# guanjq/targetdiff

Measured on NVIDIA H100. Metric: molecules/sec (1000-step sampling, CrossDocked pocket shape), higher is better.
Workload: dtype f32 (storage, LayerNorm, softmax, accumulation); GEMM operands as 2-piece bf16 splits on wgmma (3 products, ~16-bit operand mantissa)

## Files before the change

targetdiff_b200/csrc/edge_mlp_v4.cu:

```cuda
#include <stdio.h>
#include <stdlib.h>
#include <string.h>

#include "tdiff_common.cuh"
#include "hopper_mma.cuh"

namespace v4 {

constexpr int kCons = 2;
constexpr int kThreads = (kCons + 1) * 128;
constexpr int kTile = 64;
constexpr int kTabClassBytes = 2 * 128 * 128;
constexpr int kProdRegs = 40, kConsRegs = 232;
constexpr int kSrcStride = 512 + 32, kDst = 8;
constexpr int sSrc = 0, sDstRows = sSrc + kTile * kSrcStride, sMeta = sDstRows + kDst * 512, kStage = sMeta + kTile * 16;
constexpr int kMAtom = 32 * 128, kMPiece = 2 * kMAtom, kMImg = 2 * kMPiece;
template <bool FOLD>
struct Map {
  static constexpr int W = 0, T = W + 4 * 128 * 128, Par = T + (FOLD ? 1 : 2) * kTabClassBytes, X = Par + 2 * 128 * 4,
                       M = X + kCons * 4 * 2 * 128 * 4, C = M + (FOLD ? kCons * kMImg : 0), Stage = C + (FOLD ? kCons * 32 * 4 : 0),
                       Bar = Stage + kCons * kStage, Smem = Bar + 8 * (1 + 2 * kCons);
  static_assert(M % 1024 == 0 && Stage % 128 == 0 && kStage % 128 == 0 && Smem <= 227 * 1024, "shared-memory map");
};
constexpr int kOrderBar = 5;
constexpr int kFoldBar = 7;

__device__ __forceinline__ uint32_t smem_u32(const void* p) { return (uint32_t)__cvta_generic_to_shared(p); }
__device__ __forceinline__ void mbar_init(uint32_t bar, uint32_t count) {
  asm volatile("mbarrier.init.shared::cta.b64 [%0], %1;" ::"r"(bar), "r"(count) : "memory");
}
__device__ __forceinline__ void mbar_wait(uint32_t bar, uint32_t parity) {
  asm volatile(
      "{\n\t.reg .pred p;\n\tWAIT_LOOP:\n\tmbarrier.try_wait.parity.shared::cta.b64 p, [%0], %1;\n\t@p bra WAIT_DONE;\n\tbra WAIT_LOOP;\n\t"
      "WAIT_DONE:\n\t}" ::"r"(bar), "r"(parity) : "memory");
}
__device__ __forceinline__ void mbar_expect_tx(uint32_t bar, uint32_t bytes) {
  asm volatile("mbarrier.arrive.expect_tx.shared::cta.b64 _, [%0], %1;" ::"r"(bar), "r"(bytes) : "memory");
}
__device__ __forceinline__ void bulk_g2s(uint32_t smem_dst, const void* gsrc, uint32_t bytes, uint32_t bar) {
  asm volatile("cp.async.bulk.shared::cluster.global.mbarrier::complete_tx::bytes [%0], [%1], %2, [%3];" ::"r"(smem_dst), "l"(gsrc), "r"(bytes),
               "r"(bar) : "memory");
}
__device__ __forceinline__ void fence_barrier_init() { asm volatile("fence.mbarrier_init.release.cluster;" ::: "memory"); }
__device__ __forceinline__ void mbar_arrive(uint32_t bar) { asm volatile("mbarrier.arrive.shared::cta.b64 _, [%0];" ::"r"(bar) : "memory"); }
__device__ __forceinline__ void mbar_expect_tx_only(uint32_t bar, uint32_t bytes) {
  asm volatile("mbarrier.expect_tx.shared::cta.b64 [%0], %1;" ::"r"(bar), "r"(bytes) : "memory");
}
__device__ __forceinline__ void named_bar_sync(int id, int nthreads) { asm volatile("bar.sync %0, %1;" ::"r"(id), "r"(nthreads) : "memory"); }
__device__ __forceinline__ void named_bar_arrive(int id, int nthreads) { asm volatile("bar.arrive %0, %1;" ::"r"(id), "r"(nthreads) : "memory"); }
template <int N> __device__ __forceinline__ void setmaxnreg_inc() { asm volatile("setmaxnreg.inc.sync.aligned.u32 %0;" ::"n"(N)); }
template <int N> __device__ __forceinline__ void setmaxnreg_dec() { asm volatile("setmaxnreg.dec.sync.aligned.u32 %0;" ::"n"(N)); }

__device__ __forceinline__ uint32_t cvt_bf16x2(float hi, float lo) {
  uint32_t d;
  asm("cvt.rn.bf16x2.f32 %0, %1, %2;" : "=r"(d) : "f"(hi), "f"(lo));
  return d;
}
__device__ __forceinline__ float ex2_approx(float x) { float y; asm("ex2.approx.ftz.f32 %0, %1;" : "=f"(y) : "f"(x)); return y; }
__device__ __forceinline__ void stg64(float* p, float a, float b) { asm volatile("st.global.v2.f32 [%0], {%1,%2};" ::"l"(p), "f"(a), "f"(b) : "memory"); }
__device__ __forceinline__ void stg128(float* p, float a, float b, float c, float d) {
  asm volatile("st.global.v4.f32 [%0], {%1,%2,%3,%4};" ::"l"(p), "f"(a), "f"(b), "f"(c), "f"(d) : "memory");
}

struct LnParams { float b[128]; float b2[128]; float mu[20]; };
struct AggArgs {
  const float* logits;
  const float* e_w;
  float* h;
  int key_softmax;
};

template <int N, int M, int LO_BIT>
__device__ __forceinline__ void transpose_reduce(float (&t)[N], int lane) {
  if constexpr (N > M) {
    constexpr int h = (N / M / 2) << LO_BIT;
    const bool up = lane & h;
#pragma unroll
    for (int i = 0; i < N / 2; ++i) {
      const float send = up ? t[i] : t[i + N / 2];
      const float keep = up ? t[i + N / 2] : t[i];
      t[i] = keep + __shfl_xor_sync(0xffffffffu, send, h);
    }
    transpose_reduce<N / 2, M, LO_BIT>(reinterpret_cast<float(&)[N / 2]>(t), lane);
  }
}
__device__ __forceinline__ void split2(float y0, float y1, uint32_t& hi, uint32_t& lo) {
  hi = cvt_bf16x2(y1, y0);
  const float r0 = __fsub_rn(y0, __uint_as_float(hi << 16)), r1 = __fsub_rn(y1, __uint_as_float(hi & 0xffff0000u));
  lo = cvt_bf16x2(r1, r0);
}

}

using namespace v4;

template <int NOUT, bool FOLD>
__global__ void __launch_bounds__(kThreads, 1)
edge_mlp_v4_kernel(const float* __restrict__ P, int zero_row, const int* __restrict__ src, const unsigned char* __restrict__ etype,
                   const float* __restrict__ dist_arr, const int* __restrict__ row_nodes, long long n_dst, long long split_dst,
                   const int* __restrict__ d_counts, int k, int offA, int offB, const unsigned char* __restrict__ w2_image,
                   const unsigned char* __restrict__ tab_image, float coeff, const float* __restrict__ qnode, float* __restrict__ out, int out_by_slot, AggArgs agg,
                   int fold_cls, const __grid_constant__ LnParams lp) {
  static_assert(!FOLD || NOUT == 128, "the fold applies to the key MLPs");
  using L = Map<FOLD>;
  extern __shared__ __align__(1024) unsigned char smem_raw[];
  const uint32_t sbase = smem_u32(smem_raw);
  const uint32_t sW = sbase + L::W, sT = sbase + L::T, sBar = sbase + L::Bar;
  float* const s_b = reinterpret_cast<float*>(smem_raw + L::Par);
  float* const s_b2 = s_b + 128;
  const int tid = threadIdx.x, lane = tid & 31, warp = __shfl_sync(0xffffffffu, tid >> 5, 0);
  const int w = warp & 3, q = lane & 3;
  const int kshift = (k & (k - 1)) == 0 ? __ffs(k) - 1 : -1;
  auto row_dst = [&](long long idx, int& j) -> unsigned {
    const unsigned a = kshift >= 0 ? (unsigned)idx >> kshift : (unsigned)idx / (unsigned)k;
    j = (int)((unsigned)idx - a * (unsigned)k);
    return a;
  };

  if ((sbase & 1023u) != 0) __trap();
  if (d_counts) { n_dst = d_counts[0]; split_dst = d_counts[1]; }
  const long long n_rows = n_dst * k, split_rows = split_dst * k;
  long long row_lo = 0, row_hi = n_rows;
  if constexpr (FOLD) { if (fold_cls) row_lo = split_rows; else row_hi = split_rows; }
  const long long n_tiles = row_hi > row_lo ? (row_hi - row_lo + kTile - 1) / kTile : 0;
  const long long my_tiles = (n_tiles > blockIdx.x) ? (n_tiles - blockIdx.x + gridDim.x - 1) / gridDim.x : 0;
  auto full_bar = [&](int c) { return sBar + 8u * (1 + c); };
  auto empty_bar = [&](int c) { return sBar + 8u * (1 + kCons + c); };

  constexpr int kWAtom = NOUT * 128;
  constexpr int kWPiece = 2 * kWAtom;
  if (tid == 0) {
    mbar_init(sBar, 1);
    for (int c = 0; c < kCons; ++c) { mbar_init(full_bar(c), 32); mbar_init(empty_bar(c), 128); }
    fence_barrier_init();
    if constexpr (FOLD) {
      mbar_expect_tx(sBar, 4u * 128 * 128 + kTabClassBytes);
      bulk_g2s(sW, w2_image, 4u * 128 * 128, sBar);
      bulk_g2s(sT, tab_image + (size_t)fold_cls * kTabClassBytes, kTabClassBytes, sBar);
    } else {
      mbar_expect_tx(sBar, 2u * kWPiece + 2u * kTabClassBytes);
      bulk_g2s(sW, w2_image, 2u * kWPiece, sBar);
      bulk_g2s(sT, tab_image, 2u * kTabClassBytes, sBar);
    }
  }
  for (int i = tid; i < 128; i += kThreads) { s_b[i] = lp.b[i]; s_b2[i] = lp.b2[i]; }
  __syncthreads();

  if (warp < 4) {
    setmaxnreg_dec<kProdRegs>();
    if (warp >= kCons) return;
    const int c = warp;
    const uint32_t st = sbase + L::Stage + (uint32_t)c * kStage;
    for (long long it = c, use = 0; it < my_tiles; it += kCons, ++use) {
      const long long tile = blockIdx.x + it * (long long)gridDim.x, row0 = row_lo + tile * kTile;
      int j0;
      const unsigned a0 = row_dst(row0, j0);
      const long long last = (row0 + kTile - 1 < row_hi ? row0 + kTile - 1 : row_hi - 1);
      const int n_d = min(kDst, (int)(row_dst(last, j0) - a0) + 1);
      int s[2];
      int4 meta[2];
#pragma unroll
      for (int h = 0; h < 2; ++h) {
        const long long idx = row0 + lane + 32 * h;
        int jj = 0, ty = 3, slot = 0, node = -1;
        float dist = 0.f;
        s[h] = -1;
        if (idx < n_rows) {
          const unsigned a = row_dst(idx, jj);
          slot = a - a0 < (unsigned)kDst ? (int)(a - a0) + 1 : 0;
          node = row_nodes[a];
          if (node >= 0) {
            const size_t e = (size_t)node * k + jj;
            s[h] = src[e]; ty = etype[e]; dist = dist_arr[e];
          }
        }
        meta[h] = make_int4(node, s[h], __float_as_int(dist), ty | (slot << 8) | (jj << 16));
      }
      int dnode = -1;
      if (lane < n_d) dnode = row_nodes[a0 + lane];
      mbar_wait(empty_bar(c), (uint32_t)(use & 1) ^ 1u);
#pragma unroll
      for (int h = 0; h < 2; ++h) *reinterpret_cast<int4*>(smem_raw + L::Stage + c * kStage + sMeta + 16 * (lane + 32 * h)) = meta[h];
      if (lane == 0) mbar_expect_tx_only(full_bar(c), (uint32_t)(kTile + (FOLD ? 2 : 1) * n_d) * 512u);
      __syncwarp();
#pragma unroll
      for (int h = 0; h < 2; ++h)
        bulk_g2s(st + sSrc + (uint32_t)(lane + 32 * h) * kSrcStride, P + (size_t)(s[h] >= 0 ? s[h] : zero_row) * TD_NPROJ + offB, 512u, full_bar(c));
      if (lane < n_d) bulk_g2s(st + sDstRows + (uint32_t)lane * 512u, P + (size_t)(dnode >= 0 ? dnode : zero_row) * TD_NPROJ + offA, 512u, full_bar(c));
      if (FOLD && lane < n_d) bulk_g2s(st + sDstRows + (uint32_t)(2 + lane) * 512u, qnode + (size_t)(dnode >= 0 ? dnode : 0) * TD_H, 512u, full_bar(c));
      mbar_arrive(full_bar(c));
    }
    return;
  }

  setmaxnreg_inc<kConsRegs>();
  const int cwg = (warp >> 2) - 1;
  float mu[5];
#pragma unroll
  for (int m = 0; m < 5; ++m) mu[m] = lp.mu[5 * q + m];
  const float coeff2 = coeff * 1.4426950408889634f;
  mbar_wait(sBar, 0);

  const int r_base = 16 * w + (lane >> 2);
  const int pair_bar = 1 + 2 * cwg + (w >> 1);
  float* const xslot = reinterpret_cast<float*>(smem_raw + L::X) + (size_t)(cwg * 4 + w) * 256;
  float* const xpart = xslot + ((w & 1) ? -256 : 256);
  const bool do_agg = !FOLD && NOUT == 128 && qnode == nullptr && agg.logits != nullptr;
  const bool key_sm = NOUT == 128 && qnode != nullptr && agg.key_softmax;
  const unsigned char* const stage = smem_raw + L::Stage + cwg * kStage;
  const int ct = tid & 127, fu = ct & 7, fg = ct >> 3;
  const int fhd = 8 * (fg & 1) + 4 * (fu >> 2) + (fu & 3), fs = fu >> 2, frun = (fg >> 1) ^ (((fu >> 1) & 1) << 2);
  const int fn0 = 16 * ((fhd >> 1) & 1) + 2 * (fhd >> 2) + (fhd & 1);
  unsigned char* const mimg = smem_raw + L::M + cwg * kMImg;
  float* const s_c = reinterpret_cast<float*>(smem_raw + L::C) + cwg * 32;
  const int srow = k == 32 ? (w >> 1) : 0;
  const int order_mine = kOrderBar + cwg, order_other = kOrderBar + (cwg ^ 1);
  const long long n_iter = (my_tiles + kCons - 1) / kCons;
  if (n_iter == 0) return;
  if (cwg == 1) named_bar_arrive(order_other, 256);
  int set = 0;

  for (long long n = 0; n < n_iter; ++n, set ^= 1) {
    const long long it = n * kCons + cwg;
    if (it >= my_tiles) {
      for (int phase = 0; phase < 2; ++phase) { named_bar_sync(order_mine, 256); named_bar_arrive(order_other, 256); }
      continue;
    }
    const long long tile = blockIdx.x + it * (long long)gridDim.x, row0 = row_lo + tile * kTile;
    const int cls = FOLD ? 0 : (row0 >= split_rows) ? 1 : 0;
    long long idx[2];
    int node[2], s[2], ty[2], jj[2], dsl[2];
    float dist[2];
    mbar_wait(full_bar(cwg), (uint32_t)(n & 1));
#pragma unroll
    for (int h = 0; h < 2; ++h) {
      idx[h] = row0 + r_base + 8 * h;
      const int4 m4 = *reinterpret_cast<const int4*>(stage + sMeta + 16 * (r_base + 8 * h));
      node[h] = m4.x; s[h] = m4.y; dist[h] = __int_as_float(m4.z);
      ty[h] = m4.w & 0xff; dsl[h] = ((m4.w >> 8) & 0xff) - 1; jj[h] = m4.w >> 16;
    }
    float ewp[2] = {0.f, 0.f};
    float4 qf[2][2];
    if constexpr (FOLD) {
#pragma unroll
      for (int h = 0; h < 2; ++h)
        if (key_sm && idx[h] < n_rows && node[h] >= 0) ewp[h] = agg.e_w[(size_t)node[h] * k + jj[h]];
#pragma unroll
      for (int sl = 0; sl < 2; ++sl)
#pragma unroll
        for (int hf = 0; hf < 2; ++hf) {
          float4 v = make_float4(0.f, 0.f, 0.f, 0.f);
          if (sl == 0 || k == 32) {
            v = *reinterpret_cast<const float4*>(stage + sDstRows + (2 + sl) * 512 + 32 * fhd + 16 * (hf ^ fs));
            v.x *= 0.35355339059327373f; v.y *= 0.35355339059327373f; v.z *= 0.35355339059327373f; v.w *= 0.35355339059327373f;
          }
          qf[sl][hf] = v;
        }
    }
    uint32_t ghi[4][4], glo[4][4];
#pragma unroll
    for (int h = 0; h < 2; ++h) {
      const bool ok = s[h] >= 0;
      float v[8];
#pragma unroll
      for (int m = 0; m < 5; ++m) {
        const float t = dist[h] - mu[m];
        v[m] = ok ? ex2_approx(coeff2 * (t * t)) : 0.0f;
      }
      v[5] = (ok && q == 3) ? 1.0f : 0.0f;
      v[6] = v[7] = 0.0f;
      const int half = ty[h] < 2 ? 1 : 0;
#pragma unroll
      for (int kk = 0; kk < 4; ++kk)
#pragma unroll
        for (int hk = 0; hk < 2; ++hk) {
          uint32_t hi, lo;
          split2(v[4 * (kk & 1) + 2 * hk], v[4 * (kk & 1) + 2 * hk + 1], hi, lo);
          const bool own = (kk >> 1) == half;
          ghi[kk][h + 2 * hk] = own ? hi : 0u;
          glo[kk][h + 2 * hk] = own ? lo : 0u;
        }
    }
    float x[64];
#pragma unroll
    for (int h = 0; h < 2; ++h) {
      const bool valid = s[h] >= 0;
      const float* ps = reinterpret_cast<const float*>(stage + sSrc + (r_base + 8 * h) * kSrcStride) + 2 * q;
      const float* pd = (dsl[h] >= 0 ? reinterpret_cast<const float*>(stage + sDstRows + dsl[h] * 512)
                                     : P + (size_t)(valid ? node[h] : zero_row) * TD_NPROJ + offA) + 2 * q;
#pragma unroll
      for (int i = 0; i < 16; ++i) {
        const float2 b = *reinterpret_cast<const float2*>(ps + 8 * i);
        float2 a = make_float2(0.f, 0.f);
        if (valid) a = *reinterpret_cast<const float2*>(pd + 8 * i);
        x[4 * i + 2 * h] = __fadd_rn(b.x, a.x);
        x[4 * i + 2 * h + 1] = __fadd_rn(b.y, a.y);
      }
    }
    mbar_arrive(empty_bar(cwg));
    const uint32_t sTc = sT + (uint32_t)cls * kTabClassBytes;
    wgmma_fence();
    named_bar_sync(order_mine, 256);
#pragma unroll
    for (int term = 0; term < 3; ++term) {
#pragma unroll
      for (int kk = 0; kk < 4; ++kk)
        wgmma_n128_rs(x, term == 2 ? glo[kk] : ghi[kk], gmma_desc_sw128(sTc + (term == 1 ? kTabClassBytes / 2 : 0) + kk * 32),
                      1u);
    }
    wgmma_commit();
    named_bar_arrive(order_other, 256);
    if constexpr (FOLD) {
      const float* const w2s = reinterpret_cast<const float*>(smem_raw + L::W) + 8 * fhd;
#pragma unroll
      for (int jr = 0; jr < 2; ++jr) {
        const int f0 = 64 * jr + 8 * frun;
        float mv[2][8];
#pragma unroll
        for (int jf = 0; jf < 8; ++jf) {
          const float4 wa = *reinterpret_cast<const float4*>(w2s + (f0 + jf) * 128 + 4 * fs);
          const float4 wb = *reinterpret_cast<const float4*>(w2s + (f0 + jf) * 128 + 4 * (fs ^ 1));
#pragma unroll
          for (int sl = 0; sl < 2; ++sl) {
            const float4 qa = qf[sl][0], qb = qf[sl][1];
            const float pa = __fmaf_rn(wa.w, qa.w, __fmaf_rn(wa.z, qa.z, __fmaf_rn(wa.y, qa.y, wa.x * qa.x)));
            const float pb = __fmaf_rn(wb.w, qb.w, __fmaf_rn(wb.z, qb.z, __fmaf_rn(wb.y, qb.y, wb.x * qb.x)));
            mv[sl][jf] = pa + pb;
          }
        }
#pragma unroll
        for (int sl = 0; sl < 2; ++sl) {
          uint4 hi, lo;
          split2(mv[sl][0], mv[sl][1], hi.x, lo.x);
          split2(mv[sl][2], mv[sl][3], hi.y, lo.y);
          split2(mv[sl][4], mv[sl][5], hi.z, lo.z);
          split2(mv[sl][6], mv[sl][7], hi.w, lo.w);
          const int nr = fn0 + 8 * sl;
          const int off = jr * kMAtom + (nr >> 3) * 1024 + (nr & 7) * 128 + ((frun ^ (nr & 7)) << 4);
          *reinterpret_cast<uint4*>(mimg + off) = hi;
          *reinterpret_cast<uint4*>(mimg + kMPiece + off) = lo;
        }
      }
      if (fg < 2)
#pragma unroll
        for (int sl = 0; sl < 2; ++sl) {
          const float4 ba = *reinterpret_cast<const float4*>(s_b2 + 8 * fhd + 4 * fs), bb = *reinterpret_cast<const float4*>(s_b2 + 8 * fhd + 4 * (fs ^ 1));
          const float4 qa = qf[sl][0], qb = qf[sl][1];
          const float pa = __fmaf_rn(ba.w, qa.w, __fmaf_rn(ba.z, qa.z, __fmaf_rn(ba.y, qa.y, ba.x * qa.x)));
          const float pb = __fmaf_rn(bb.w, qb.w, __fmaf_rn(bb.z, qb.z, __fmaf_rn(bb.y, qb.y, bb.x * qb.x)));
          s_c[16 * sl + fhd] = pa + pb;
        }
      asm volatile("fence.proxy.async.shared::cta;" ::: "memory");
    }
    wgmma_wait_all();
    float rstd[2];
#pragma unroll
    for (int h = 0; h < 2; ++h) {
      float qa = 0.f, qb = 0.f;
#pragma unroll
      for (int i = 0; i < 16; ++i) {
        qa = __fmaf_rn(x[4 * i + 2 * h], x[4 * i + 2 * h], qa);
        qb = __fmaf_rn(x[4 * i + 2 * h + 1], x[4 * i + 2 * h + 1], qb);
      }
      float var = qa + qb;
      var += __shfl_xor_sync(0xffffffffu, var, 1);
      var += __shfl_xor_sync(0xffffffffu, var, 2);
      rstd[h] = rsqrtf(var * (1.0f / 128.0f) + 1e-5f);
    }
    uint32_t ahi[8][4], alo[8][4];
#pragma unroll
    for (int kk = 0; kk < 8; ++kk)
#pragma unroll
      for (int r = 0; r < 4; ++r) {
        const int h = r & 1, col = 16 * kk + 8 * (r >> 1) + 2 * q, e = 8 * kk + 2 * r;
        const float2 b = *reinterpret_cast<const float2*>(s_b + col);
        const float y0 = __fmaf_rn(x[e], rstd[h], b.x), y1 = __fmaf_rn(x[e + 1], rstd[h], b.y);
        split2(fmaxf(y0, 0.f), fmaxf(y1, 0.f), ahi[kk][r], alo[kk][r]);
      }
    float o[NOUT / 2];
    if constexpr (FOLD) {
      named_bar_sync(kFoldBar + cwg, 128);
#pragma unroll
      for (int sl = 0; sl < 2; ++sl) {
        const float4 cv = *reinterpret_cast<const float4*>(s_c + 16 * sl + 4 * q);
#pragma unroll
        for (int h = 0; h < 2; ++h) {
          o[4 * sl + 2 * h] = cv.x; o[4 * sl + 2 * h + 1] = cv.y;
          o[4 * (2 + sl) + 2 * h] = cv.z; o[4 * (2 + sl) + 2 * h + 1] = cv.w;
        }
      }
    }
    wgmma_fence();
    named_bar_sync(order_mine, 256);
#pragma unroll
    for (int term = 0; term < 3; ++term) {
#pragma unroll
      for (int kk = 0; kk < 8; ++kk) {
        if constexpr (FOLD) {
          const uint64_t desc = gmma_desc_sw128(sbase + L::M + cwg * kMImg + (term == 1 ? kMPiece : 0) + (kk >> 2) * kMAtom + (kk & 3) * 32);
          wgmma_n32_rs(reinterpret_cast<float(&)[16]>(o), term == 2 ? alo[kk] : ahi[kk], desc, 1u);
        } else {
          const uint64_t desc = gmma_desc_sw128(sW + (term == 1 ? kWPiece : 0) + (kk >> 2) * kWAtom + (kk & 3) * 32);
          if constexpr (NOUT == 128) wgmma_n128_rs(o, term == 2 ? alo[kk] : ahi[kk], desc, (term | kk) ? 1u : 0u);
          else wgmma_n16_rs(o, term == 2 ? alo[kk] : ahi[kk], desc, (term | kk) ? 1u : 0u);
        }
      }
    }
    wgmma_commit();
    named_bar_arrive(order_other, 256);
    wgmma_wait_all();

    long long orow[2];
    bool owrite[2];
#pragma unroll
    for (int h = 0; h < 2; ++h) {
      orow[h] = out_by_slot ? ((long long)node[h] * k + jj[h]) : idx[h];
      owrite[h] = idx[h] < n_rows && node[h] >= 0;
    }
    if constexpr (NOUT == 16) {
#pragma unroll
      for (int h = 0; h < 2; ++h)
        if (owrite[h])
#pragma unroll
          for (int i = 0; i < 2; ++i) {
            const float2 bb = *reinterpret_cast<const float2*>(s_b2 + 8 * i + 2 * q);
            stg64(out + (size_t)orow[h] * 16 + 8 * i + 2 * q, o[4 * i + 2 * h] + bb.x, o[4 * i + 2 * h + 1] + bb.y);
          }
    } else if (do_agg) {
      const long long dslot = tile * 2 + (w >> 1);
      const int dnode = dslot < n_dst ? row_nodes[dslot] : -1;
      const bool active = dnode >= 0;
      const int ccol = 64 * (w & 1) + 2 * lane;
      float2 hin = make_float2(0.f, 0.f);
      if (active) hin = *reinterpret_cast<const float2*>(agg.h + (size_t)dnode * TD_H + ccol);
      float wt[2][16];
#pragma unroll
      for (int h = 0; h < 2; ++h)
#pragma unroll
        for (int i = 0; i < 4; ++i) {
          float4 t4 = make_float4(0.f, 0.f, 0.f, 0.f);
          if (active) t4 = __ldg(reinterpret_cast<const float4*>(agg.logits + (size_t)idx[h] * TD_HEADS + 4 * i));
          wt[h][4 * i] = t4.x; wt[h][4 * i + 1] = t4.y; wt[h][4 * i + 2] = t4.z; wt[h][4 * i + 3] = t4.w;
        }
      float t[32];
#pragma unroll
      for (int i = 0; i < 16; ++i) {
        const float2 bb = *reinterpret_cast<const float2*>(s_b2 + 8 * i + 2 * q);
#pragma unroll
        for (int c = 0; c < 2; ++c) {
          const float b = c ? bb.y : bb.x;
          t[2 * i + c] = __fadd_rn(__fmul_rn(__fadd_rn(o[4 * i + c], b), wt[0][i]), __fmul_rn(__fadd_rn(o[4 * i + 2 + c], b), wt[1][i]));
        }
      }
      transpose_reduce<32, 4, 2>(t, lane);
      float* slot = xslot + 128 * set;
      const int c0 = 16 * (lane >> 2) + 2 * q;
      *reinterpret_cast<float2*>(slot + c0) = make_float2(t[0], t[1]);
      *reinterpret_cast<float2*>(slot + c0 + 8) = make_float2(t[2], t[3]);
      named_bar_sync(pair_bar, 64);
      if (active) {
        const float* se = ((w & 1) ? xpart : xslot) + 128 * set;
        const float* so = ((w & 1) ? xslot : xpart) + 128 * set;
        const float2 a = *reinterpret_cast<const float2*>(se + ccol), b = *reinterpret_cast<const float2*>(so + ccol);
        *reinterpret_cast<float2*>(agg.h + (size_t)dnode * TD_H + ccol) = make_float2(hin.x + (a.x + b.x), hin.y + (a.y + b.y));
      }
    } else if (!FOLD && qnode == nullptr) {
#pragma unroll
      for (int h = 0; h < 2; ++h)
        if (owrite[h])
#pragma unroll
          for (int i = 0; i < 16; ++i) {
            const float2 bb = *reinterpret_cast<const float2*>(s_b2 + 8 * i + 2 * q);
            stg64(out + (size_t)orow[h] * 128 + 8 * i + 2 * q, o[4 * i + 2 * h] + bb.x, o[4 * i + 2 * h + 1] + bb.y);
          }
    } else {
      float lg[32];
      if constexpr (FOLD) {
#pragma unroll
        for (int h = 0; h < 2; ++h)
#pragma unroll
          for (int u = 0; u < 4; ++u) {
            const int e0 = 4 * (2 * (u >> 1)) + 2 * h + (u & 1);
            lg[4 * h + u] = srow ? o[e0 + 4] : o[e0];
          }
      } else {
#pragma unroll
        for (int h = 0; h < 2; ++h) {
          const float* qrow = qnode + (size_t)(node[h] >= 0 ? node[h] : 0) * TD_H + 2 * q;
#pragma unroll
          for (int i = 0; i < 16; ++i) {
            const float2 qv = __ldg(reinterpret_cast<const float2*>(qrow + 8 * i));
            const float2 bb = *reinterpret_cast<const float2*>(s_b2 + 8 * i + 2 * q);
            lg[8 * (i >> 2) + 4 * h + (i & 3)] = __fmaf_rn(o[4 * i + 2 * h + 1] + bb.y, qv.y, (o[4 * i + 2 * h] + bb.x) * qv.x);
          }
        }
        transpose_reduce<32, 8, 0>(lg, lane);
#pragma unroll
        for (int u = 0; u < 8; ++u) lg[u] *= 0.35355339059327373f;
      }
      if (key_sm) {
        bool valid_e[2];
        float ew[2];
#pragma unroll
        for (int h = 0; h < 2; ++h) {
          valid_e[h] = false; ew[h] = 0.f;
          if (owrite[h]) {
            valid_e[h] = s[h] >= 0;
            ew[h] = FOLD ? ewp[h] : agg.e_w[(size_t)node[h] * k + jj[h]];
          }
        }
        float mx[4], sm[4];
#pragma unroll
        for (int u = 0; u < 4; ++u) {
          lg[u] = valid_e[0] ? lg[u] * 1.4426950408889634f : -INFINITY;
          lg[4 + u] = valid_e[1] ? lg[4 + u] * 1.4426950408889634f : -INFINITY;
          mx[u] = fmaxf(lg[u], lg[4 + u]);
#pragma unroll
          for (int m = 4; m < 32; m <<= 1) mx[u] = fmaxf(mx[u], __shfl_xor_sync(0xffffffffu, mx[u], m));
        }
        if (lane < 4) *reinterpret_cast<float4*>(xslot + 4 * q) = make_float4(mx[0], mx[1], mx[2], mx[3]);
        named_bar_sync(pair_bar, 64);
        const float4 pm = *reinterpret_cast<const float4*>(xpart + 4 * q);
        mx[0] = fmaxf(mx[0], pm.x); mx[1] = fmaxf(mx[1], pm.y); mx[2] = fmaxf(mx[2], pm.z); mx[3] = fmaxf(mx[3], pm.w);
#pragma unroll
        for (int u = 0; u < 4; ++u) {
          lg[u] = valid_e[0] ? ex2_approx(lg[u] - mx[u]) : 0.0f;
          lg[4 + u] = valid_e[1] ? ex2_approx(lg[4 + u] - mx[u]) : 0.0f;
          sm[u] = lg[u] + lg[4 + u];
#pragma unroll
          for (int m = 4; m < 32; m <<= 1) sm[u] += __shfl_xor_sync(0xffffffffu, sm[u], m);
        }
        if (lane < 4) *reinterpret_cast<float4*>(xslot + 128 + 4 * q) = make_float4(sm[0], sm[1], sm[2], sm[3]);
        named_bar_sync(pair_bar, 64);
        const float4 ps = *reinterpret_cast<const float4*>(xpart + 128 + 4 * q);
        const float pl[4] = {ps.x, ps.y, ps.z, ps.w};
#pragma unroll
        for (int u = 0; u < 4; ++u) {
          const float l = sm[u] + pl[u];
          const float inv = l > 0.0f ? 1.0f / l : 0.0f;
          lg[u] = lg[u] * ew[0] * inv;
          lg[4 + u] = lg[4 + u] * ew[1] * inv;
        }
#pragma unroll
        for (int h = 0; h < 2; ++h)
          if (idx[h] < n_rows) stg128(out + (size_t)idx[h] * TD_HEADS + 4 * q, lg[4 * h], lg[4 * h + 1], lg[4 * h + 2], lg[4 * h + 3]);
      } else {
#pragma unroll
        for (int h = 0; h < 2; ++h)
          if (owrite[h]) stg128(out + (size_t)orow[h] * TD_HEADS + 4 * q, lg[4 * h], lg[4 * h + 1], lg[4 * h + 2], lg[4 * h + 3]);
      }
    }
  }
  if (cwg == 0) named_bar_sync(order_mine, 256);
}

void td_launch_edge_mlp_v4(const float* P, int zero_row, const int* src, const unsigned char* etype, const float* dist, const int* row_nodes, long long n_dst,
                           long long split_dst, const int* d_counts, int k, const TdMlp& m, const float* h_offsets, float coeff,
                           const float* h_ln_b, const float* h_b2, const float* qnode, float* out, int out_by_slot,
                           const float* agg_logits, const float* agg_e_w, float* agg_h, int key_softmax, int sm_count, cudaStream_t st) {
  if (n_dst == 0) return;
  LnParams lp;
  memcpy(lp.b, h_ln_b, sizeof(lp.b));
  memset(lp.b2, 0, sizeof(lp.b2));
  memcpy(lp.b2, h_b2, sizeof(float) * (size_t)m.nout);
  memcpy(lp.mu, h_offsets, sizeof(lp.mu));
  static size_t opted128[TD_MAX_DEVICES] = {0}, opted16[TD_MAX_DEVICES] = {0}, optedF[TD_MAX_DEVICES] = {0};
  td_opt_in_smem(edge_mlp_v4_kernel<128, false>, Map<false>::Smem, opted128);
  td_opt_in_smem(edge_mlp_v4_kernel<16, false>, Map<false>::Smem, opted16);
  td_opt_in_smem(edge_mlp_v4_kernel<128, true>, Map<true>::Smem, optedF);
  auto grid_of = [&](long long n_dst_range) {
    const long long n_tiles = (n_dst_range * k + kTile - 1) / kTile;
    return (int)(n_tiles < sm_count ? n_tiles : sm_count);
  };
  AggArgs agg = {agg_logits, agg_e_w, agg_h, (key_softmax && k == 32) ? 1 : 0};
  if (m.nout == 16) {
    edge_mlp_v4_kernel<16, false><<<grid_of(n_dst), kThreads, Map<false>::Smem, st>>>(
        P, zero_row, src, etype, dist, row_nodes, n_dst, split_dst, d_counts, k, m.offA, m.offB, m.w2_img, m.tabcls_img, coeff, nullptr, out,
        out_by_slot, agg, 0, lp);
  } else if (qnode && (k == 32 || k == 64)) {
    const long long n_cls[2] = {split_dst, n_dst - split_dst};
    for (int cls = 0; cls < 2; ++cls)
      if (n_cls[cls] > 0)
        edge_mlp_v4_kernel<128, true><<<grid_of(n_cls[cls]), kThreads, Map<true>::Smem, st>>>(
            P, zero_row, src, etype, dist, row_nodes, n_dst, split_dst, d_counts, k, m.offA, m.offB,
            reinterpret_cast<const unsigned char*>(m.w2t), m.tabcls_img, coeff, qnode, out, out_by_slot, agg, cls, lp);
  } else {
    edge_mlp_v4_kernel<128, false><<<grid_of(n_dst), kThreads, Map<false>::Smem, st>>>(
        P, zero_row, src, etype, dist, row_nodes, n_dst, split_dst, d_counts, k, m.offA, m.offB, m.w2_img, m.tabcls_img, coeff, qnode, out,
        out_by_slot, agg, 0, lp);
  }
}
```

Before: 18.16.

## Use three consumer warpgroups for the non-fold 128-wide edge MLP, split launches by class

Makes the consumer count a per-template parameter: the non-fold 128-output kernel now runs three consumer warpgroups with a smaller register budget (160 per consumer thread) and drops the ordered named-barrier handoff between consumers. Every variant is now launched once per class, so only one class's table is loaded into shared memory, and the freed space pays for the extra stage. The goal is more edge tiles in flight and better latency hiding. The cost is that the tighter register cap may cause spills, and wgmma issue from three groups is no longer serialized. The doubled launches add overhead, and the aggregation path now reads the destination node from per-row metadata instead of row_nodes.

```diff
diff --git a/targetdiff_b200/csrc/edge_mlp_v4.cu b/targetdiff_b200/csrc/edge_mlp_v4.cu
--- a/targetdiff_b200/csrc/edge_mlp_v4.cu
+++ b/targetdiff_b200/csrc/edge_mlp_v4.cu
@@ -7,23 +7,25 @@
 
 namespace v4 {
 
-constexpr int kCons = 2;
-constexpr int kThreads = (kCons + 1) * 128;
 constexpr int kTile = 64;
 constexpr int kTabClassBytes = 2 * 128 * 128;
-constexpr int kProdRegs = 40, kConsRegs = 232;
 constexpr int kSrcStride = 512 + 32, kDst = 8;
 constexpr int sSrc = 0, sDstRows = sSrc + kTile * kSrcStride, sMeta = sDstRows + kDst * 512, kStage = sMeta + kTile * 16;
 constexpr int kMAtom = 32 * 128, kMPiece = 2 * kMAtom, kMImg = 2 * kMPiece;
-template <bool FOLD>
+template <int NOUT, bool FOLD>
 struct Map {
-  static constexpr int W = 0, T = W + 4 * 128 * 128, Par = T + (FOLD ? 1 : 2) * kTabClassBytes, X = Par + 2 * 128 * 4,
+  static constexpr int kCons = (NOUT == 128 && !FOLD) ? 3 : 2;
+  static constexpr int kThreads = (kCons + 1) * 128;
+  static constexpr int kProdRegs = kCons == 3 ? 32 : 40, kConsRegs = kCons == 3 ? 160 : 232;
+  static constexpr int W = 0, T = W + 4 * 128 * 128, Par = T + kTabClassBytes, X = Par + 2 * 128 * 4,
                        M = X + kCons * 4 * 2 * 128 * 4, C = M + (FOLD ? kCons * kMImg : 0), Stage = C + (FOLD ? kCons * 32 * 4 : 0),
                        Bar = Stage + kCons * kStage, Smem = Bar + 8 * (1 + 2 * kCons);
+  static constexpr bool kOrdered = kCons == 2;
+  static constexpr int kPairBar = 1, kOrderBar = kPairBar + 2 * kCons, kFoldBar = kOrderBar + kCons;
   static_assert(M % 1024 == 0 && Stage % 128 == 0 && kStage % 128 == 0 && Smem <= 227 * 1024, "shared-memory map");
+  static_assert(128 * kProdRegs + kCons * 128 * kConsRegs == kThreads * (65536 / kThreads / 8 * 8), "register split");
+  static_assert(kFoldBar + kCons <= 16, "named barriers");
 };
-constexpr int kOrderBar = 5;
-constexpr int kFoldBar = 7;
 
 __device__ __forceinline__ uint32_t smem_u32(const void* p) { return (uint32_t)__cvta_generic_to_shared(p); }
 __device__ __forceinline__ void mbar_init(uint32_t bar, uint32_t count) {
@@ -95,14 +97,15 @@
 using namespace v4;
 
 template <int NOUT, bool FOLD>
-__global__ void __launch_bounds__(kThreads, 1)
+__global__ void __launch_bounds__(Map<NOUT, FOLD>::kThreads, 1)
 edge_mlp_v4_kernel(const float* __restrict__ P, int zero_row, const int* __restrict__ src, const unsigned char* __restrict__ etype,
                    const float* __restrict__ dist_arr, const int* __restrict__ row_nodes, long long n_dst, long long split_dst,
                    const int* __restrict__ d_counts, int k, int offA, int offB, const unsigned char* __restrict__ w2_image,
                    const unsigned char* __restrict__ tab_image, float coeff, const float* __restrict__ qnode, float* __restrict__ out, int out_by_slot, AggArgs agg,
-                   int fold_cls, const __grid_constant__ LnParams lp) {
+                   int cls, const __grid_constant__ LnParams lp) {
   static_assert(!FOLD || NOUT == 128, "the fold applies to the key MLPs");
-  using L = Map<FOLD>;
+  using L = Map<NOUT, FOLD>;
+  constexpr int kCons = L::kCons, kThreads = L::kThreads;
   extern __shared__ __align__(1024) unsigned char smem_raw[];
   const uint32_t sbase = smem_u32(smem_raw);
   const uint32_t sW = sbase + L::W, sT = sbase + L::T, sBar = sbase + L::Bar;
@@ -120,8 +123,7 @@
   if ((sbase & 1023u) != 0) __trap();
   if (d_counts) { n_dst = d_counts[0]; split_dst = d_counts[1]; }
   const long long n_rows = n_dst * k, split_rows = split_dst * k;
-  long long row_lo = 0, row_hi = n_rows;
-  if constexpr (FOLD) { if (fold_cls) row_lo = split_rows; else row_hi = split_rows; }
+  const long long row_lo = cls ? split_rows : 0, row_hi = cls ? n_rows : split_rows;
   const long long n_tiles = row_hi > row_lo ? (row_hi - row_lo + kTile - 1) / kTile : 0;
   const long long my_tiles = (n_tiles > blockIdx.x) ? (n_tiles - blockIdx.x + gridDim.x - 1) / gridDim.x : 0;
   auto full_bar = [&](int c) { return sBar + 8u * (1 + c); };
@@ -129,25 +131,20 @@
 
   constexpr int kWAtom = NOUT * 128;
   constexpr int kWPiece = 2 * kWAtom;
+  constexpr uint32_t kWBytes = FOLD ? 4u * 128 * 128 : 2u * kWPiece;
   if (tid == 0) {
     mbar_init(sBar, 1);
     for (int c = 0; c < kCons; ++c) { mbar_init(full_bar(c), 32); mbar_init(empty_bar(c), 128); }
     fence_barrier_init();
-    if constexpr (FOLD) {
-      mbar_expect_tx(sBar, 4u * 128 * 128 + kTabClassBytes);
-      bulk_g2s(sW, w2_image, 4u * 128 * 128, sBar);
-      bulk_g2s(sT, tab_image + (size_t)fold_cls * kTabClassBytes, kTabClassBytes, sBar);
-    } else {
-      mbar_expect_tx(sBar, 2u * kWPiece + 2u * kTabClassBytes);
-      bulk_g2s(sW, w2_image, 2u * kWPiece, sBar);
-      bulk_g2s(sT, tab_image, 2u * kTabClassBytes, sBar);
-    }
+    mbar_expect_tx(sBar, kWBytes + kTabClassBytes);
+    bulk_g2s(sW, w2_image, kWBytes, sBar);
+    bulk_g2s(sT, tab_image + (size_t)cls * kTabClassBytes, kTabClassBytes, sBar);
   }
   for (int i = tid; i < 128; i += kThreads) { s_b[i] = lp.b[i]; s_b2[i] = lp.b2[i]; }
   __syncthreads();
 
   if (warp < 4) {
-    setmaxnreg_dec<kProdRegs>();
+    setmaxnreg_dec<L::kProdRegs>();
     if (warp >= kCons) return;
     const int c = warp;
     const uint32_t st = sbase + L::Stage + (uint32_t)c * kStage;
@@ -193,7 +190,7 @@
     return;
   }
 
-  setmaxnreg_inc<kConsRegs>();
+  setmaxnreg_inc<L::kConsRegs>();
   const int cwg = (warp >> 2) - 1;
   float mu[5];
 #pragma unroll
@@ -202,7 +199,7 @@
   mbar_wait(sBar, 0);
 
   const int r_base = 16 * w + (lane >> 2);
-  const int pair_bar = 1 + 2 * cwg + (w >> 1);
+  const int pair_bar = L::kPairBar + 2 * cwg + (w >> 1);
   float* const xslot = reinterpret_cast<float*>(smem_raw + L::X) + (size_t)(cwg * 4 + w) * 256;
   float* const xpart = xslot + ((w & 1) ? -256 : 256);
   const bool do_agg = !FOLD && NOUT == 128 && qnode == nullptr && agg.logits != nullptr;
@@ -214,20 +211,22 @@
   unsigned char* const mimg = smem_raw + L::M + cwg * kMImg;
   float* const s_c = reinterpret_cast<float*>(smem_raw + L::C) + cwg * 32;
   const int srow = k == 32 ? (w >> 1) : 0;
-  const int order_mine = kOrderBar + cwg, order_other = kOrderBar + (cwg ^ 1);
+  const int order_mine = L::kOrderBar + cwg, order_next = L::kOrderBar + (cwg + 1) % kCons;
+  auto order_wait = [&] { if constexpr (L::kOrdered) named_bar_sync(order_mine, 256); };
+  auto order_pass = [&] { if constexpr (L::kOrdered) named_bar_arrive(order_next, 256); };
   const long long n_iter = (my_tiles + kCons - 1) / kCons;
   if (n_iter == 0) return;
-  if (cwg == 1) named_bar_arrive(order_other, 256);
+  if (cwg == kCons - 1) order_pass();
   int set = 0;
 
   for (long long n = 0; n < n_iter; ++n, set ^= 1) {
     const long long it = n * kCons + cwg;
     if (it >= my_tiles) {
-      for (int phase = 0; phase < 2; ++phase) { named_bar_sync(order_mine, 256); named_bar_arrive(order_other, 256); }
+      if constexpr (L::kOrdered)
+        for (int phase = 0; phase < 2; ++phase) { order_wait(); order_pass(); }
       continue;
     }
-    const long long tile = blockIdx.x + it * (long long)gridDim.x, row0 = row_lo + tile * kTile;
-    const int cls = FOLD ? 0 : (row0 >= split_rows) ? 1 : 0;
+    const long long row0 = row_lo + (blockIdx.x + it * (long long)gridDim.x) * kTile;
     long long idx[2];
     int node[2], s[2], ty[2], jj[2], dsl[2];
     float dist[2];
@@ -298,18 +297,17 @@
       }
     }
     mbar_arrive(empty_bar(cwg));
-    const uint32_t sTc = sT + (uint32_t)cls * kTabClassBytes;
     wgmma_fence();
-    named_bar_sync(order_mine, 256);
+    order_wait();
 #pragma unroll
     for (int term = 0; term < 3; ++term) {
 #pragma unroll
       for (int kk = 0; kk < 4; ++kk)
-        wgmma_n128_rs(x, term == 2 ? glo[kk] : ghi[kk], gmma_desc_sw128(sTc + (term == 1 ? kTabClassBytes / 2 : 0) + kk * 32),
+        wgmma_n128_rs(x, term == 2 ? glo[kk] : ghi[kk], gmma_desc_sw128(sT + (term == 1 ? kTabClassBytes / 2 : 0) + kk * 32),
                       1u);
     }
     wgmma_commit();
-    named_bar_arrive(order_other, 256);
+    order_pass();
     if constexpr (FOLD) {
       const float* const w2s = reinterpret_cast<const float*>(smem_raw + L::W) + 8 * fhd;
 #pragma unroll
@@ -379,7 +377,7 @@
       }
     float o[NOUT / 2];
     if constexpr (FOLD) {
-      named_bar_sync(kFoldBar + cwg, 128);
+      named_bar_sync(L::kFoldBar + cwg, 128);
 #pragma unroll
       for (int sl = 0; sl < 2; ++sl) {
         const float4 cv = *reinterpret_cast<const float4*>(s_c + 16 * sl + 4 * q);
@@ -391,7 +389,7 @@
       }
     }
     wgmma_fence();
-    named_bar_sync(order_mine, 256);
+    order_wait();
 #pragma unroll
     for (int term = 0; term < 3; ++term) {
 #pragma unroll
@@ -407,7 +405,7 @@
       }
     }
     wgmma_commit();
-    named_bar_arrive(order_other, 256);
+    order_pass();
     wgmma_wait_all();
 
     long long orow[2];
@@ -427,8 +425,7 @@
             stg64(out + (size_t)orow[h] * 16 + 8 * i + 2 * q, o[4 * i + 2 * h] + bb.x, o[4 * i + 2 * h + 1] + bb.y);
           }
     } else if (do_agg) {
-      const long long dslot = tile * 2 + (w >> 1);
-      const int dnode = dslot < n_dst ? row_nodes[dslot] : -1;
+      const int dnode = node[0];
       const bool active = dnode >= 0;
       const int ccol = 64 * (w & 1) + 2 * lane;
       float2 hin = make_float2(0.f, 0.f);
@@ -551,7 +548,7 @@
       }
     }
   }
-  if (cwg == 0) named_bar_sync(order_mine, 256);
+  if (cwg == 0) order_wait();
 }
 
 void td_launch_edge_mlp_v4(const float* P, int zero_row, const int* src, const unsigned char* etype, const float* dist, const int* row_nodes, long long n_dst,
@@ -565,28 +562,27 @@
   memcpy(lp.b2, h_b2, sizeof(float) * (size_t)m.nout);
   memcpy(lp.mu, h_offsets, sizeof(lp.mu));
   static size_t opted128[TD_MAX_DEVICES] = {0}, opted16[TD_MAX_DEVICES] = {0}, optedF[TD_MAX_DEVICES] = {0};
-  td_opt_in_smem(edge_mlp_v4_kernel<128, false>, Map<false>::Smem, opted128);
-  td_opt_in_smem(edge_mlp_v4_kernel<16, false>, Map<false>::Smem, opted16);
-  td_opt_in_smem(edge_mlp_v4_kernel<128, true>, Map<true>::Smem, optedF);
-  auto grid_of = [&](long long n_dst_range) {
-    const long long n_tiles = (n_dst_range * k + kTile - 1) / kTile;
-    return (int)(n_tiles < sm_count ? n_tiles : sm_count);
-  };
+  td_opt_in_smem(edge_mlp_v4_kernel<128, false>, Map<128, false>::Smem, opted128);
+  td_opt_in_smem(edge_mlp_v4_kernel<16, false>, Map<16, false>::Smem, opted16);
+  td_opt_in_smem(edge_mlp_v4_kernel<128, true>, Map<128, true>::Smem, optedF);
   AggArgs agg = {agg_logits, agg_e_w, agg_h, (key_softmax && k == 32) ? 1 : 0};
-  if (m.nout == 16) {
-    edge_mlp_v4_kernel<16, false><<<grid_of(n_dst), kThreads, Map<false>::Smem, st>>>(
-        P, zero_row, src, etype, dist, row_nodes, n_dst, split_dst, d_counts, k, m.offA, m.offB, m.w2_img, m.tabcls_img, coeff, nullptr, out,
-        out_by_slot, agg, 0, lp);
-  } else if (qnode && (k == 32 || k == 64)) {
-    const long long n_cls[2] = {split_dst, n_dst - split_dst};
-    for (int cls = 0; cls < 2; ++cls)
-      if (n_cls[cls] > 0)
-        edge_mlp_v4_kernel<128, true><<<grid_of(n_cls[cls]), kThreads, Map<true>::Smem, st>>>(
-            P, zero_row, src, etype, dist, row_nodes, n_dst, split_dst, d_counts, k, m.offA, m.offB,
-            reinterpret_cast<const unsigned char*>(m.w2t), m.tabcls_img, coeff, qnode, out, out_by_slot, agg, cls, lp);
-  } else {
-    edge_mlp_v4_kernel<128, false><<<grid_of(n_dst), kThreads, Map<false>::Smem, st>>>(
-        P, zero_row, src, etype, dist, row_nodes, n_dst, split_dst, d_counts, k, m.offA, m.offB, m.w2_img, m.tabcls_img, coeff, qnode, out,
-        out_by_slot, agg, 0, lp);
+  const bool fold = m.nout == 128 && qnode && (k == 32 || k == 64);
+  const long long n_cls[2] = {split_dst, n_dst - split_dst};
+  for (int cls = 0; cls < 2; ++cls) {
+    if (n_cls[cls] == 0) continue;
+    const long long n_tiles = (n_cls[cls] * k + kTile - 1) / kTile;
+    const int grid = (int)(n_tiles < sm_count ? n_tiles : sm_count);
+    if (m.nout == 16)
+      edge_mlp_v4_kernel<16, false><<<grid, Map<16, false>::kThreads, Map<16, false>::Smem, st>>>(
+          P, zero_row, src, etype, dist, row_nodes, n_dst, split_dst, d_counts, k, m.offA, m.offB, m.w2_img, m.tabcls_img, coeff, nullptr,
+          out, out_by_slot, agg, cls, lp);
+    else if (fold)
+      edge_mlp_v4_kernel<128, true><<<grid, Map<128, true>::kThreads, Map<128, true>::Smem, st>>>(
+          P, zero_row, src, etype, dist, row_nodes, n_dst, split_dst, d_counts, k, m.offA, m.offB,
+          reinterpret_cast<const unsigned char*>(m.w2t), m.tabcls_img, coeff, qnode, out, out_by_slot, agg, cls, lp);
+    else
+      edge_mlp_v4_kernel<128, false><<<grid, Map<128, false>::kThreads, Map<128, false>::Smem, st>>>(
+          P, zero_row, src, etype, dist, row_nodes, n_dst, split_dst, d_counts, k, m.offA, m.offB, m.w2_img, m.tabcls_img, coeff, qnode,
+          out, out_by_slot, agg, cls, lp);
   }
 }
```

Result: faster. 18.94 (median of 6 runs) (+4.3%).
